# leonardsiegert/PULPo

Measured on AMD Instinct MI355X. Metric: volume-pairs/sec fwd+bwd, 160^3 fp32, higher is better.
Workload: dtype f32

## Files before the change

### include/pulpo_hip.h

```cpp
#ifndef PULPO_HIP_H
#define PULPO_HIP_H

#include <stddef.h>
#include <stdint.h>

#ifdef __cplusplus
extern "C" {
#endif

#define PULPO_ABI_VERSION 8
int pulpo_abi_version(void);
const char* pulpo_last_error(void);

size_t pulpo_conv3d_k3_packed_floats(int K, int N);
int pulpo_conv3d_k3_pack_weight(const float* w , float* wp, int Cin, int Cout, int dgrad, void* stream);
int pulpo_conv3d_k3_stat_tiles(int B, int D, int H, int W);
int pulpo_conv3d_k3_tile_config(int K, int N);
size_t pulpo_conv3d_k3_fwd_scratch_floats(int B, int D, int H, int W, int K, int N);
int pulpo_conv3d_k3_fwd(const float* in, int64_t in_bs, int64_t in_ps, int64_t in_cs, const float* wp, const float* bias, float* out,
                        int64_t out_bs, int64_t out_ps, int64_t out_cs, float* stats, float* scratch , int B,
                        int D, int H, int W, int K, int N, void* stream);
int pulpo_conv3d_k3_fwd_bn_lrelu(const float* in, int64_t in_bs, int64_t in_ps, int64_t in_cs, const float* wp, const float* bias,
                                 const float* coef, float slope, float* out, int64_t out_bs, int64_t out_ps, int64_t out_cs, float* scratch, int B,
                                 int D, int H, int W, int K, int N, void* stream);
// ... 68 lines not shown
int pulpo_heads_bwd_blocks(int B, int64_t V, int C);
int pulpo_heads_bwd(const float* h, int64_t ps, const float* Wt, const float* g0, const float* g1, const float* g2, const float* eps,
                    const float* sigma, float* dh, int64_t dps, float* partial , int nout, int B, int64_t V, int C,
                    void* stream);

int pulpo_avgpool2_fwd(const float* in, int64_t ips, float* out, int64_t ops, int B, int D, int H, int W, int C, void* stream);
int pulpo_avgpool2_bwd(const float* gout, int64_t gops, float* gin, int64_t gips, int B, int D, int H, int W, int C, void* stream);
int pulpo_avgpool2_bwd_add(const float* gout, int64_t gops, const float* add, int64_t aps, float* gin, int64_t gips, int B, int D, int H, int W,
                           int C, void* stream);
int pulpo_resize_trilinear_fwd(const float* in, const float* add, float* out, int64_t nplanes, int Di, int Hi, int Wi, int Do, int Ho, int Wo,
                               float mult, void* stream);
int pulpo_resize_trilinear_bwd(const float* gout, float* gin, int64_t nplanes, int Di, int Hi, int Wi, int Do, int Ho, int Wo, float mult,
                               void* stream);
int pulpo_resize_trilinear_scaled_fwd(const float* in, const float* add, float* out, int64_t nplanes, int Di, int Hi, int Wi, int Do, int Ho,
                                      int Wo, float scale_d, float scale_h, float scale_w, float mult, void* stream);
int pulpo_resize_trilinear_scaled_bwd(const float* gout, float* gin, int64_t nplanes, int Di, int Hi, int Wi, int Do, int Ho, int Wo,
                                      float scale_d, float scale_h, float scale_w, float mult, void* stream);
int pulpo_feedback_up2_fwd(const float* const* srcs , const int* chans , int nsrc, float* out, int64_t ops,
                           int B, int Di, int Hi, int Wi, void* stream);
int pulpo_feedback_up2_bwd(const float* gout, int64_t gops, float* const* gsrcs , const int* chans, int nsrc,
                           int B, int Di, int Hi, int Wi, void* stream);

int pulpo_warp3d_fwd(const float* df, const float* img, float* out, int B, int C, int Dg, int Hg, int Wg, int Di, int Hi, int Wi, void* stream);
int pulpo_warp_mask_fwd(const float* df, const float* mask, float* out, int B, int Dg, int Hg, int Wg, int Di, int Hi, int Wi, void* stream);
int pulpo_warp3d_bwd(const float* df, const float* img, const float* gout, float* gdf, float* gimg, int B, int C, int Dg, int Hg, int Wg, int Di,
                     int Hi, int Wi, void* stream);
int pulpo_vecint_fwd(const float* v, float* work, int B, int D, int H, int W, int nsteps, void* stream);
size_t pulpo_vecint_bwd_tmp_floats(int B, int D, int H, int W, int nsteps);
int pulpo_vecint_bwd(const float* work, const float* gout, float* gin, float* tmp , int B, int D, int H, int W,
                     int nsteps, void* stream);

int pulpo_loss_blocks(int64_t n);
int pulpo_ncc_fwd(const float* I, const float* J, float* S , float* T , float* partial, int B, int D, int H, int W,
                  int win, void* stream);
int pulpo_ncc_bwd(const float* I, const float* J, const float* S, float* T , const float* gscale, float coef, float* gJ, int B, int D,
                  int H, int W, int win, void* stream);
int pulpo_ncc_masked_fwd(const float* I, const float* J, const float* wa, const float* wb , float* S ,
                         float* T , float* partial , int B, int D, int H, int W, int win, void* stream);
int pulpo_ncc_masked_bwd(const float* I, const float* J, const float* S, const float* wa, const float* wb , float* T ,
                         const float* gscale, float coef, float* gJ, int B, int D, int H, int W, int win, void* stream);
int pulpo_masked_finish(const float* partial, int nblk, double scale, int root, double count, float* out , void* stream);
int pulpo_mind_blocks(int B, int D, int H, int W, int d);
int pulpo_mind_descriptor(const float* I, float* out , int B, int D, int H, int W, int d, float eps, void* stream);
int pulpo_mind_fwd(const float* y_true, const float* y_pred, const float* wa , const float* wb , float* partial, int B, int D,
                   int H, int W, int d, float eps, void* stream);
int pulpo_mind_bwd(const float* y_true, const float* y_pred, const float* wa , const float* wb , float* scratch ,
                   const float* gscale, float coef, float* gpred, int B, int D, int H, int W, int d, float eps, void* stream);
int pulpo_kl_fwd(const float* mu, const float* sigma, const float* mu1 , const float* sigma1 , int64_t n,
                 float* partial, void* stream);
int pulpo_kl_bwd(const float* mu, const float* sigma, const float* mu1, const float* sigma1, const float* gscale, float coef, float* gmu,
                 float* gsigma, int64_t n, void* stream);
int pulpo_l2reg_fwd(const float* df, int64_t nplanes, int D, int H, int W, float* partial, void* stream);
int pulpo_l2reg_bwd(const float* df, const float* gscale, float coef, float* gdf, int64_t nplanes, int D, int H, int W, void* stream);
int pulpo_bending_blocks(int64_t nplanes, int D, int H, int W);
int pulpo_bending_fwd(const float* df, int64_t nplanes, int D, int H, int W, float* partial, void* stream);
int pulpo_bending_bwd(const float* df, const float* gscale, float coef, float* gdf, int64_t nplanes, int D, int H, int W, void* stream);
int pulpo_weighted_sum_fwd(const float* terms, const float* weights, int n, float scale, int scaled, float* levels, float* total, void* stream);
int pulpo_weighted_sum_bwd(const float* gtotal, const float* glevels, const float* weights, int n, float scale, float* gterms, void* stream);

int pulpo_metric_blocks(int64_t n);
int pulpo_sqdiff_fwd(const float* a, const float* b, int64_t n, float* partial, void* stream);
int pulpo_sqdiff_bwd(const float* a, const float* b, const float* gscale, float coef, float* ga, int64_t n, void* stream);
int pulpo_sqdiff_masked_fwd(const float* a, const float* b, const float* wa, const float* wb ,
                            float* partial , int B, int C, int64_t V, void* stream);
int pulpo_sqdiff_masked_bwd(const float* a, const float* b, const float* wa, const float* wb , const float* gscale, float coef, float* ga,
                            int B, int C, int64_t V, void* stream);
int pulpo_dice_blocks(int64_t V);
int pulpo_dice_fwd(const float* inp, const float* tgt, int nplanes, int64_t V, float dice_factor, float* partial, double* numden, float* loss,
                   void* stream);
int pulpo_dice_bwd(const float* inp, const float* tgt, const double* numden, const float* gscale, int nplanes, int64_t V, float dice_factor,
                   float* ginp, void* stream);
int pulpo_jacdet_fwd(const float* df, float* out, double* partial , int B, int D, int H, int W, int normalize, void* stream);
int pulpo_jdetstd_finalize(const double* partial, int64_t n, float lamb, double* stat, float* loss, void* stream);
int pulpo_kl_nondiag_fwd(const float* mu, const float* sigma, int64_t nplanes, int D, int H, int W, float prior_lambda, float* partial, float* loss,
                         void* stream);
int pulpo_kl_nondiag_bwd(const float* mu, const float* sigma, const float* gscale, int64_t nplanes, int D, int H, int W, float prior_lambda,
                         float* gmu, float* gsigma, void* stream);
int pulpo_jdetstd_bwd(const float* df, const float* jdet, const double* stat, const float* gscale, float lamb, float* gdf, int B, int D, int H, int W,
                      int normalize, void* stream);

int pulpo_rmse(const float* a, const float* b, int64_t n, float* partial , float* out, void* stream);
int pulpo_dsc(const float* inp, const float* tgt, int nplanes, int64_t V, float* partial , float* out,
              void* stream);
int pulpo_percent_leq0(const float* x, int64_t n, float* partial , float* out, void* stream);
int pulpo_warp_landmarks(const float* lm , const float* df , float* out , int nlm, int nsamp,
                         int nd, int D, int H, int W, int* flag, void* stream);
int pulpo_field_quality_blocks(int B, int D, int H, int W);
size_t pulpo_field_quality_ws_bytes(int B, int D, int H, int W);
int pulpo_field_quality(const float* df, float* out , void* ws, int B, int D, int H, int W, int normalize, void* stream);

size_t pulpo_vecint_pair_scratch_floats(int B, int D, int H, int W, int nsteps);
int pulpo_vecint_pair_fwd(const float* v, float* fwd, float* inv, float* scratch , int B, int D, int H, int W, int nsteps,
                          void* stream);
size_t pulpo_inverse_consistency_ws_bytes(int B, int D, int H, int W);
int pulpo_inverse_consistency(const float* a, const float* b, float* out , void* ws, int B, int D, int H, int W, void* stream);
int pulpo_transport_points(const float* pts , const float* field , float* out , int npts,
                           int nsamp, int nd, int D, int H, int W, int* flag, void* stream);

int pulpo_affine_field(const float* theta, float* out, int B, int D, int H, int W, void* stream);
int pulpo_affine_warp_fwd(const float* theta, const float* img, float* out, int B, int C, int Dg, int Hg, int Wg, int Di, int Hi, int Wi, void* stream);
size_t pulpo_affine_warp_bwd_ws_bytes(int B, int Dg, int Hg, int Wg);
int pulpo_affine_warp_bwd(const float* theta, const float* img, const float* gout, float* gtheta , void* ws, int B, int C, int Dg, int Hg,
                          int Wg, int Di, int Hi, int Wi, void* stream);
int pulpo_affine_compose(const float* theta, const float* df, float* out, int B, int Dg, int Hg, int Wg, int Di, int Hi, int Wi, void* stream);

int pulpo_mc_moments_update(const float* sample, float* mean, float* m2, int64_t n, int k, void* stream);
int pulpo_mc_moments_std(const float* m2, const float* scale , float* out , int B, int C, int64_t V, int k, void* stream);

size_t pulpo_warp_labels_ws_bytes(int B, int C);
int pulpo_warp_labels(const float* df, const void* labels, int ldt, int C, const void* target , float* onehot ,
                      void* amax , float* dice , float* mean , float* m2 ,
                      int k, void* ws, int* flag, int B, int Dg, int Hg, int Wg, int Di, int Hi, int Wi, void* stream);
int pulpo_labels_check(const void* labels, int ldt, int64_t n, int C, int* flag, void* stream);
int pulpo_warp_labels_soft_dice(const float* df, const void* labels, const void* target, int ldt, int C, float* dice, float* mean, void* ws,
                                int* flag, int B, int Dg, int Hg, int Wg, int Di, int Hi, int Wi, int Dt, int Ht, int Wt, void* stream);
int pulpo_labels_from_onehot(const float* seg, void* labels, int ldt, int B, int C, int64_t V, void* stream);
int pulpo_map_ncc_blocks(int64_t n);
int pulpo_map_ncc(const float* a, const float* b, int64_t n, double* partial, double* out, void* stream);
int pulpo_label_dice_fwd(const float* df, const void* labels, const void* target, int ldt, int C, float dice_factor, float* loss, float* dice,
                         float* coef, void* ws, int* flag, int B, int Dg, int Hg, int Wg, int Di, int Hi, int Wi, int Dt, int Ht, int Wt,
                         void* stream);
int pulpo_label_dice_bwd(const float* df, const void* labels, const void* target, int ldt, int C, const float* coef, const float* gup, float* ddf,
                         int B, int Dg, int Hg, int Wg, int Di, int Hi, int Wi, int Dt, int Ht, int Wt, void* stream);
int pulpo_labels_pool2(const void* labels, int ldt, int C, float* out, int B, int D, int H, int W, void* stream);
int pulpo_labels_resize(const void* labels, int ldt, int C, float* out, int B, int Dt, int Ht, int Wt, int Do, int Ho, int Wo, void* stream);

#define PULPO_EDT_INF (1 << 29)
int pulpo_edt_sq(const void* mask, int* out, int B, int D, int H, int W, void* stream);
int64_t pulpo_surface_distances_bins(int D, int H, int W);
size_t pulpo_surface_distances_ws_bytes(int B, int C, int D, int H, int W);
int pulpo_surface_distances(const void* lab_a, const void* lab_b, int ldt, int C, double q, float* out, int* hist , void* ws, int* flag,
                            int B, int D, int H, int W, int nd, void* stream);

int pulpo_augment_apply(const float* theta, const float* phi, int spacing, int Gz, int Gy, int Gx, const float* img, float* img_out, int C,
                        const float* mask, float* mask_out, int Cm, const void* labels, void* labels_out, int ldt, const float* iparams, int iflags,
                        const float* bias, int Lz, int Ly, int Lx, const void* seed, float fill, int fill_label, int B, int D, int H, int W,
                        void* stream);
int pulpo_bspline_field(const float* phi, const float* theta, float* out, int spacing, int Gz, int Gy, int Gx, int B, int D, int H, int W, void* stream);
int pulpo_philox4x32(const void* counters, const void* key, void* out, int64_t n, void* stream);

int pulpo_adam_step(float* p, const float* g, float* m, float* v, int64_t n, float lr, double beta1, double beta2, float eps, int step, float gscale,
                    void* stream);
int pulpo_anchored_adam_step(float* p, const float* g, float* m, float* v, const float* mean, const float* prec, int64_t n, float lr, double beta1,
                             double beta2, float eps, int step, float* partial, void* stream);

size_t pulpo_conv3d_k3_packed_wino3_floats(int K, int N);
int pulpo_conv3d_k3_pack_weight_wino3(const float* w , float* wp, int Cin, int Cout, int dgrad, void* stream);
int pulpo_conv3d_k3_fwd_wino3(const float* in, int64_t in_bs, int64_t in_ps, int64_t in_cs, const float* wp, const float* bias, const float* coef,
                              float slope, float* out, int64_t out_bs, int64_t out_ps, int64_t out_cs, float* stats, int B, int D, int H, int W, int K,
                              int N, void* stream);
int pulpo_conv3d_k3_dgrad_wino3_bnred(const float* in, int64_t in_bs, int64_t in_ps, int64_t in_cs, const float* wp, float* out, int64_t out_bs,
                                      int64_t out_ps, const float* bn_y, int64_t bn_y_bs, int64_t bn_y_ps, const float* bn_coef, float slope, float* part,
                                      int B, int D, int H, int W, int K, int N, void* stream);

int pulpo_conv3d_k3_fwd_bf16_t(const void* in, int64_t in_bs, int64_t in_ps, int64_t in_cs, const uint16_t* wp, const float* bias, void* out,
                               int64_t out_bs, int64_t out_ps, int64_t out_cs, int dt, float* stats, float* scratch, int B, int D, int H, int W,
                               int K, int N, void* stream);
int pulpo_conv3d_k3_fwd_bn_lrelu_bf16_t(const void* in, int64_t in_bs, int64_t in_ps, int64_t in_cs, const uint16_t* wp, const float* bias,
                                        const float* coef, float slope, void* out, int64_t out_bs, int64_t out_ps, int64_t out_cs, int dt,
                                        float* scratch, int B, int D, int H, int W, int K, int N, void* stream);
int pulpo_conv3d_k3_wgrad_bf16_t(const void* in, int64_t in_bs, int64_t in_ps, int64_t in_cs, const void* dy, int64_t dy_bs, int64_t dy_ps,
                                 int64_t dy_cs, int dt, float* dw, int accumulate, float* scratch, int B, int D, int H, int W, int Cin, int Cout,
                                 void* stream);
int pulpo_bn_lrelu_apply_t(const void* y, int y_dt, int64_t yps, void* z, int z_dt, int64_t zps, const float* coef, int64_t npix, int C, float slope,
                           void* stream);
int pulpo_bn_lrelu_apply_pool2_t(const void* y, int y_dt, int64_t yps, void* z , int z_dt, int64_t zps,
                                 void* pooled , int64_t pps,
                                 const float* coef, int B, int D, int H, int W, int C, float slope, void* stream);
int pulpo_bn_lrelu_bwd_reduce_t(const void* dz, int dz_dt, int64_t dzps, const void* y, int y_dt, int64_t yps, const float* coef, int64_t npix, int C,
                                float slope, float* partial, void* stream);
int pulpo_bn_lrelu_bwd_apply_t(const void* dz, int dz_dt, int64_t dzps, const void* y, int y_dt, int64_t yps, const float* coef, const double* totd,
                               void* dy , int64_t dyps, int64_t npix, int C, float slope, float* partial2, void* stream);
int pulpo_avgpool2_bwd_bnred_t(const void* gout, int64_t gops, const void* add, int64_t aps, void* gin, int64_t gips, int g_dt ,
                               const void* y, int y_dt, int64_t yps, const float* coef, float slope, float* partial, int B, int D, int H, int W,
                               int C, void* stream);
int pulpo_heads_fwd_t(const void* h, int h_dt, int64_t ps, const float* Wt, const float* bias, const float* eps, float* o0, float* o1, float* o2,
                      int nout, int B, int64_t V, int C, void* stream);
int pulpo_heads_bwd_t(const void* h, int h_dt, int64_t ps, const float* Wt, const float* g0, const float* g1, const float* g2, const float* eps,
                      const float* sigma, void* dh , int64_t dps, float* partial, int nout, int B, int64_t V, int C, void* stream);
int pulpo_avgpool2_fwd_t(const void* in, int64_t ips, void* out, int64_t ops, int dt, int B, int D, int H, int W, int C, void* stream);
int pulpo_avgpool2_bwd_t(const void* gout, int64_t gops, const void* add , int64_t aps, void* gin, int64_t gips, int dt, int B, int D,
                         int H, int W, int C, void* stream);
int pulpo_feedback_up2_fwd_t(const float* const* srcs , const int* chans , int nsrc, void* out,
                             int dt, int64_t ops, int B, int Di, int Hi, int Wi, void* stream);
int pulpo_feedback_up2_bwd_t(const void* gout, int dt, int64_t gops, float* const* gsrcs , const int* chans,
                             int nsrc, int B, int Di, int Hi, int Wi, void* stream);

int pulpo_conv3d_k3_wgrad_bn_rows(int B, int D, int H, int W, int Cout);
int pulpo_conv3d_k3_wgrad_bn(const float* in, int64_t in_bs, int64_t in_ps, int64_t in_cs, const void* dz, int dz_dt, int64_t dz_bs, int64_t dz_ps,
                             const float* y, int64_t y_bs, int64_t y_ps, const float* coef, const double* totd, float slope, float* dw,
                             int accumulate, float* scratch, float* part2, int B, int D, int H, int W, int Cin, int Cout, void* stream);

int pulpo_bn_lrelu_bwd_apply_pooled_t(const void* gout, int64_t gops, const void* add , int64_t aps, int g_dt, const void* y, int y_dt,
                                      int64_t yps, const float* coef, const double* totd, void* dy , int64_t dyps, float slope,
                                      float* partial2, int B, int D, int H, int W, int C, void* stream);

int pulpo_bn_lrelu_apply_kb(const float* y, int64_t yps, float* z, int64_t zps, int64_t zkb, const float* coef, int64_t npix, int C, float slope, void* stream);
int pulpo_bn_lrelu_bwd_apply_kb_t(const void* dz, int dz_dt, int64_t dzps, int64_t dzkb, const float* y, int64_t yps, const float* coef, const double* totd,
                                  float* dy, int64_t dyps, int64_t dykb, int64_t npix, int C, float slope, float* partial2, void* stream);
int pulpo_conv3d_k3_wgrad_bn_kb(const float* in, int64_t in_bs, int64_t in_ps, int64_t in_cs, const float* dz, int64_t dz_bs, int64_t dz_ps, int64_t dz_kb,
                                const float* y, int64_t y_bs, int64_t y_ps, const float* coef, const double* totd, float slope, float* dw, int accumulate,
                                float* scratch, float* part2, int B, int D, int H, int W, int Cin, int Cout, void* stream);
int pulpo_bn_lrelu_bwd_apply_pooled_kb_t(const void* gout, int64_t gops, const void* add , int64_t aps, int g_dt, const float* y, int64_t yps,
                                         const float* coef, const double* totd, float* dy, int64_t dyps, int64_t dykb, float slope, float* partial2,
                                         int B, int D, int H, int W, int C, void* stream);
int pulpo_conv3d_k3_fwd_wino3_kb(const float* in, int64_t in_bs, int64_t in_ps, int64_t in_kb, const float* wp, const float* bias, const float* coef,
                                 float slope, float* out, int64_t out_bs, int64_t out_ps, int64_t out_kb, float* stats, int B, int D, int H, int W, int K,
                                 int N, void* stream);
int pulpo_conv3d_k3_dgrad_wino3_bnred_kb(const float* in, int64_t in_bs, int64_t in_ps, int64_t in_kb, const float* wp, float* out, int64_t out_bs,
                                         int64_t out_ps, int64_t out_kb, const float* bn_y, int64_t bn_y_bs, int64_t bn_y_ps, const float* bn_coef, float slope,
                                         float* part, int B, int D, int H, int W, int K, int N, void* stream);
int pulpo_conv3d_k3_wgrad_kb(const float* in, int64_t in_bs, int64_t in_ps, int64_t in_kb, const float* dy, int64_t dy_bs, int64_t dy_ps, int64_t dy_kb,
                             float* dw, int accumulate, float* scratch, float* slabs , int nslab, int B, int D, int H, int W, int Cin, int Cout,
                             void* stream);

int pulpo_conv3d_k3_wgrad_det_slabs(int Cin, int Cout);
int pulpo_conv3d_k3_wgrad_det(const float* in, int64_t in_bs, int64_t in_ps, int64_t in_cs, const float* dy, int64_t dy_bs, int64_t dy_ps,
                              int64_t dy_cs, float* dw, int accumulate, float* scratch, float* slabs, int nslab, int B, int D, int H, int W,
                              int Cin, int Cout, void* stream);
int pulpo_conv3d_k3_wgrad_bf16_det_t(const void* in, int64_t in_bs, int64_t in_ps, int64_t in_cs, const void* dy, int64_t dy_bs, int64_t dy_ps,
                                     int64_t dy_cs, int dt, float* dw, int accumulate, float* scratch, float* slabs, int nslab, int B, int D,
                                     int H, int W, int Cin, int Cout, void* stream);
int pulpo_resize_trilinear_scaled_bwd_det(const float* gout, float* gin, int64_t nplanes, int Di, int Hi, int Wi, int Do, int Ho, int Wo,
                                          float scale_d, float scale_h, float scale_w, float mult, void* stream);
size_t pulpo_warp3d_bwd_det_ws_bytes(int B, int C, int Di, int Hi, int Wi);
int pulpo_warp3d_bwd_det(const float* df, const float* img, const float* gout, float* gdf , float* gimg ,
                         void* ws , int B, int C, int Dg, int Hg, int Wg, int Di, int Hi, int Wi, void* stream);
size_t pulpo_vecint_bwd_det_ws_bytes(int B, int D, int H, int W, int nsteps);
int pulpo_vecint_bwd_det(const float* work, const float* gout, float* gin, void* ws , int B, int D, int H, int W,
                         int nsteps, void* stream);

int pulpo_conv3d_k3_wgrad_grid(int B, int D, int H, int W, int Cin, int Cout, int max_workgroups);
int pulpo_conv3d_k3_wgrad_wg(const float* in, int64_t in_bs, int64_t in_ps, int64_t in_cs, const float* dy, int64_t dy_bs, int64_t dy_ps,
                             int64_t dy_cs, float* dw, int accumulate, float* scratch, int B, int D, int H, int W, int Cin, int Cout, void* stream,
                             int max_workgroups);
int pulpo_conv3d_k3_wgrad_det_wg(const float* in, int64_t in_bs, int64_t in_ps, int64_t in_cs, const float* dy, int64_t dy_bs, int64_t dy_ps,
                                 int64_t dy_cs, float* dw, int accumulate, float* scratch, float* slabs, int nslab, int B, int D, int H, int W,
                                 int Cin, int Cout, void* stream, int max_workgroups);
int pulpo_conv3d_k3_wgrad_kb_wg(const float* in, int64_t in_bs, int64_t in_ps, int64_t in_kb, const float* dy, int64_t dy_bs, int64_t dy_ps, int64_t dy_kb,
                                float* dw, int accumulate, float* scratch, float* slabs , int nslab, int B, int D, int H, int W, int Cin, int Cout,
                                void* stream, int max_workgroups);

int pulpo_heads_fwd_bn_t(const float* y, int64_t ps, const float* coef, float slope, const float* Wt, const float* bias, const float* eps ,
                         float* o0, float* o1, float* o2, int nout, int B, int64_t V, int C, void* stream);
int pulpo_heads_bwd_bn_t(const float* y, int64_t ps, const float* coef, float slope, const float* Wt, const float* g0, const float* g1, const float* g2,
                         const float* eps, const float* sigma, float* partial , float* bnpart , int nout, int B,
                         int64_t V, int C, void* stream);
int pulpo_bn_lrelu_bwd_apply_heads_t(const float* y, int64_t yps, const float* coef, const double* totd, float slope, const float* Wt, const float* g0,
                                     const float* g1, const float* g2, const float* eps, const float* sigma, float* dy, int64_t dyps, float* partial2,
                                     int nout, int B, int64_t V, int C, void* stream);
int pulpo_bn_lrelu_bwd_apply_heads_kb_t(const float* y, int64_t yps, const float* coef, const double* totd, float slope, const float* Wt, const float* g0,
                                        const float* g1, const float* g2, const float* eps, const float* sigma, float* dy, int64_t dyps, int64_t dykb,
                                        float* partial2, int nout, int B, int64_t V, int C, void* stream);

#ifdef __cplusplus
}
#endif
#endif
```

### pulpo_amd/ops.py

```python
from __future__ import annotations

import collections
import contextlib
import ctypes
import os
from typing import Optional, Sequence, Tuple

import torch

from ._lib import PulpoHipError, lib

CL = torch.channels_last_3d
LRELU_SLOPE = 0.2


def _ptr(t: Optional[torch.Tensor]):
    return None if t is None else ctypes.c_void_p(t.data_ptr())


def _stream():
    return ctypes.c_void_p(torch.cuda.current_stream().cuda_stream)


def _require_gpu(*ts: Optional[torch.Tensor], act: bool = False):
# ... 164 lines not shown
    if n > 2 and not _sampled():
        return None
    ev = torch.cuda.Event(enable_timing=True)
    ev.record()
    return ev


def _hbm_end(start, name: str, nbytes: float):
    if start is None or HBM_TRACE is None:
        return
    end = torch.cuda.Event(enable_timing=True)
    end.record()
    HBM_TRACE.append((name, nbytes, start, end))


def _trace_end(start, name: str, flops: float, nbytes: float = 0.0):
    if start is None:
        return
    end = torch.cuda.Event(enable_timing=True)
    end.record()
    CONV_TRACE.append((name, flops, start, end, nbytes))


CONV_PRECISION = "fp32"
ACT_BF16 = False
CONV_ALGO = None


def set_conv_precision(precision: str, activations: str = "fp32") -> None:
    global CONV_PRECISION, ACT_BF16
    if precision not in ("fp32", "bf16"):
        raise ValueError(f"conv precision is {precision}. Not a known option.")
    if activations not in ("fp32", "bf16") or (activations == "bf16" and precision != "bf16"):
        raise ValueError(f"activation storage is {activations} with {precision} operands. Not a known option.")
    CONV_PRECISION = precision
    ACT_BF16 = activations == "bf16"


def act_dtype():
    return torch.bfloat16 if ACT_BF16 else torch.float32


DETERMINISTIC = os.environ.get("PULPO_DETERMINISTIC", "0") == "1"


def set_deterministic(on: bool = True) -> None:
    global DETERMINISTIC
    DETERMINISTIC = bool(on)


BN_REDUCE_IN_DGRAD = True
FUSE_INPUT_WGRAD = True
POOLED_BN_BACKWARD = True
FUSE_HEAD_BN = True


def _use_bf16(K: int) -> bool:
    return CONV_PRECISION == "bf16" and K > 4


_WEIGHT_EPOCH = 0


def invalidate_weight_packs() -> None:
    global _WEIGHT_EPOCH
    _WEIGHT_EPOCH += 1
    _PACK_REGISTRY.clear()


_PACK_REGISTRY: dict = {}
_PACK_TABLES: dict = {}
_UNREFRESHABLE_PACKS = False
_registrations = 0


def _register_pack(w: torch.Tensor, wp: torch.Tensor, Cin: int, Cout: int, dgrad: bool, kind: int) -> None:
    global _registrations
    import weakref
    _PACK_REGISTRY[id(wp)] = (weakref.ref(w), wp, Cin, Cout, dgrad, kind)
    _registrations += 1
    if _registrations % 64 == 0:
        for k in [k for k, e in _PACK_REGISTRY.items() if e[0]() is None]:
            del _PACK_REGISTRY[k]


def refresh_weight_packs() -> None:
    global _UNREFRESHABLE_PACKS
    if _UNREFRESHABLE_PACKS or not _PACK_REGISTRY:
        _UNREFRESHABLE_PACKS = False
        invalidate_weight_packs()
        return
    jobs = []
    device = None
    for key, (wref, wp, Cin, Cout, dgrad, kind) in list(_PACK_REGISTRY.items()):
        w = wref()
        cache = getattr(w, "_pulpo_packs", None) if w is not None else None
        if cache is None or cache[0] != (w._version, w.data_ptr(), _WEIGHT_EPOCH) or not any(v is wp for v in cache[1].values()):
            del _PACK_REGISTRY[key]
            continue
        jobs.append((w.data_ptr(), wp.data_ptr(), Cin, Cout, int(dgrad), kind))
        device = w.device
    if not jobs:
        invalidate_weight_packs()
        return
    tkey = tuple(jobs)
    table = _PACK_TABLES.get(tkey)
    if table is None:
        import struct
        raw = b"".join(struct.pack("<QQiiii", *job) for job in tkey)
        table = torch.frombuffer(bytearray(raw), dtype=torch.uint8).to(device)
        if len(_PACK_TABLES) > 4:
            _PACK_TABLES.clear()
        _PACK_TABLES[tkey] = table
    lib.call("pulpo_conv3d_k3_pack_weights_multi", _ptr(table), len(tkey), _stream())


def _pack_weight(w: torch.Tensor, dgrad: bool, shape=None, both: bool = False) -> torch.Tensor:
    if not w.is_leaf:
        return _pack_weight_now(w, dgrad, shape, register=False)
    cache = getattr(w, "_pulpo_packs", None)
    ver = (w._version, w.data_ptr(), _WEIGHT_EPOCH)
    if cache is None or cache[0] != ver:
        cache = (ver, {})
        try:
            w._pulpo_packs = cache
        except AttributeError:
            return _pack_weight_now(w, dgrad, shape, register=False)
    def key(d):
        return (d, CONV_PRECISION, CONV_ALGO, None if shape is None else tuple(shape))
    if both and key(not dgrad) not in cache[1]:
        cache[1][key(not dgrad)] = _pack_weight_now(w, not dgrad, shape)
    if key(dgrad) not in cache[1]:
        cache[1][key(dgrad)] = _pack_weight_now(w, dgrad, shape)
    return cache[1][key(dgrad)]


def _pack_weight_now(w: torch.Tensor, dgrad: bool, shape=None, register: bool = True) -> torch.Tensor:
    Cout, Cin = w.shape[0], w.shape[1]
    K, N = (Cout, Cin) if dgrad else (Cin, Cout)
    global _UNREFRESHABLE_PACKS
    if _use_bf16(K):
        wp = torch.empty(lib.query("pulpo_conv3d_k3_packed_bf16_elems", K, N), device=w.device, dtype=torch.int16)
        lib.call("pulpo_conv3d_k3_pack_weight_bf16", _ptr(w.contiguous()), _ptr(wp), Cin, Cout, int(dgrad), _stream())
        wp._pulpo_algo = "bf16"
        if register:
            if w.is_contiguous():
                _register_pack(w, wp, Cin, Cout, dgrad, 3)
            else:
                _UNREFRESHABLE_PACKS = True
        return wp
    algo = lib.query("pulpo_conv3d_k3_algo", *shape, K, N) if shape is not None else 0
    if CONV_ALGO is not None and algo != 0:
        algo = {"direct": 0, "wino2": 2, "wino3": algo}[CONV_ALGO]
    if algo == 3:
        wp = torch.empty(lib.query("pulpo_conv3d_k3_packed_wino3_floats", K, N), device=w.device, dtype=torch.float32)
        lib.call("pulpo_conv3d_k3_pack_weight_wino3", _ptr(w.contiguous()), _ptr(wp), Cin, Cout, int(dgrad), _stream())
        wp._pulpo_algo = "wino3"
        if register:
            if w.is_contiguous():
                _register_pack(w, wp, Cin, Cout, dgrad, 4)
            else:
                _UNREFRESHABLE_PACKS = True
        return wp
    if algo == 2:
        wp = torch.empty(lib.query("pulpo_conv3d_k3_packed_wino2_floats", K, N), device=w.device, dtype=torch.float32)
        lib.call("pulpo_conv3d_k3_pack_weight_wino2", _ptr(w.contiguous()), _ptr(wp), Cin, Cout, int(dgrad), _stream())
        wp._pulpo_algo = "wino2"
        if register:
            if w.is_contiguous():
                _register_pack(w, wp, Cin, Cout, dgrad, 2)
            else:
                _UNREFRESHABLE_PACKS = True
        return wp
    wp = torch.empty(lib.query("pulpo_conv3d_k3_packed_floats", K, N), device=w.device, dtype=torch.float32)
    lib.call("pulpo_conv3d_k3_pack_weight", _ptr(w.contiguous()), _ptr(wp), Cin, Cout, int(dgrad), _stream())
    wp._pulpo_algo = "direct"
    if register:
        if w.is_contiguous():
            _register_pack(w, wp, Cin, Cout, dgrad, 0)
        else:
            _UNREFRESHABLE_PACKS = True
    return wp


def _conv_raw(x: torch.Tensor, wp: torch.Tensor, bias: Optional[torch.Tensor], out: torch.Tensor, K: int, N: int,
              stats: Optional[torch.Tensor], coef: Optional[torch.Tensor] = None):
    B, _, D, H, W = _dims5(x)
    ob, op, oc = (0, 0, 1) if is_blocked(out) else grid_strides(out)
    algo = getattr(wp, "_pulpo_algo", "bf16" if wp.dtype == torch.int16 else "direct")
    if isinstance(x, _BlockedGrad) or is_blocked(x) or is_blocked(out):
        xt, xb_, xp_, xkb, xblk = _opnd(x)
        ot, ob_, op_, okb, oblk = _opnd(out)
        if algo != "wino3" or (not oblk and not _vec4(out)) or (not xblk and grid_strides(x)[2] != 1):
            raise PulpoHipError("conv3d on channel-blocked tensors: F(2x2x2,3x3x3) kernel, channels-last or blocked fp32 operands only")
        t0 = _trace_begin()
        lib.call("pulpo_conv3d_k3_fwd_wino3_kb", _ptr(xt), xb_, xp_, xkb, _ptr(wp), _ptr(bias), _ptr(coef), LRELU_SLOPE, _ptr(ot), ob_, op_, okb, _ptr(stats),
                 B, D, H, W, K, N, _stream())
        _trace_end(t0, "conv3d_k3_wino3_mfma<false>", 54.0 * K * N * B * D * H * W, 4.0 * (K + N) * B * D * H * W)
        return
    xb, xp, xc = grid_strides(x)
    bf16 = algo == "bf16"
    vec_ok = _vec4(x, K)
    if algo == "wino3":
        if not vec_ok:
            x = _packed_cl(x)
            xb, xp, xc = grid_strides(x)
        if not _vec4(out):
            raise PulpoHipError("conv3d (F(2x2x2,3x3x3) kernel): the result must be channels-last and 16-byte aligned")
        t0 = _trace_begin()
        lib.call("pulpo_conv3d_k3_fwd_wino3", _ptr(x), xb, xp, xc, _ptr(wp), _ptr(bias), _ptr(coef), LRELU_SLOPE, _ptr(out), ob, op, oc, _ptr(stats),
                 B, D, H, W, K, N, _stream())
        _trace_end(t0, "conv3d_k3_wino3_mfma<false>", 54.0 * K * N * B * D * H * W, 4.0 * (K + N) * B * D * H * W)
        return
    if algo == "wino2":
        if (D % 4 or D * H * W < 8000) and not vec_ok:
            x = _packed_cl(x)
            xb, xp, xc = grid_strides(x)
            vec_ok = True
        nscr = lib.query("pulpo_conv3d_k3_fwd_wino2_scratch_floats", B, D, H, W, K, N)
        scratch = torch.empty(nscr, device=x.device, dtype=torch.float32) if nscr else None
        t0 = _trace_begin()
        lib.call("pulpo_conv3d_k3_fwd_wino2", _ptr(x), xb, xp, xc, _ptr(wp), _ptr(bias), _ptr(coef), LRELU_SLOPE, _ptr(out), ob, op, oc, _ptr(stats),
                 _ptr(scratch), B, D, H, W, K, N, _stream())
        kname = f"conv3d_k3_wino2_mfma<{'true' if vec_ok else 'false'}>"
        if vec_ok and t0 is not None and lib.query("pulpo_conv3d_k3_wino2_pipelined", D, H, W, K, xp):
            kname = "conv3d_k3_wino2p_mfma<false>"
        _trace_end(t0, kname, 54.0 * K * N * B * D * H * W, 4.0 * (K + N) * B * D * H * W)
        return
    sfx = "_bf16" if bf16 else ""
    nscr = lib.query(f"pulpo_conv3d_k3_fwd{sfx}_scratch_floats", B, D, H, W, K, N)
    scratch = torch.empty(nscr, device=x.device, dtype=torch.float32) if nscr else None
    t0 = _trace_begin()
    if bf16:
        if x.dtype != out.dtype:
            raise PulpoHipError(f"conv3d (bf16 operands): input {x.dtype} and output {out.dtype} must share one storage type")
        if coef is None:
            lib.call("pulpo_conv3d_k3_fwd_bf16_t", _ptr(x), xb, xp, xc, _ptr(wp), _ptr(bias), _ptr(out), ob, op, oc, _dt(x), _ptr(stats), _ptr(scratch),
                     B, D, H, W, K, N, _stream())
        else:
            lib.call("pulpo_conv3d_k3_fwd_bn_lrelu_bf16_t", _ptr(x), xb, xp, xc, _ptr(wp), _ptr(bias), _ptr(coef), LRELU_SLOPE, _ptr(out), ob, op, oc,
                     _dt(x), _ptr(scratch), B, D, H, W, K, N, _stream())
    elif coef is None:
        lib.call("pulpo_conv3d_k3_fwd", _ptr(x), xb, xp, xc, _ptr(wp), _ptr(bias), _ptr(out), ob, op, oc, _ptr(stats), _ptr(scratch), B, D, H,
                 W, K, N, _stream())
    else:
        lib.call("pulpo_conv3d_k3_fwd_bn_lrelu", _ptr(x), xb, xp, xc, _ptr(wp), _ptr(bias), _ptr(coef), LRELU_SLOPE, _ptr(out), ob, op, oc,
                 _ptr(scratch), B, D, H, W, K, N, _stream())
    if t0 is not None:
        if bf16:
            name = f"conv3d_k3_mfma_bf16<{64 if N % 64 == 0 else 32},{'true' if vec_ok else 'false'}>"
        else:
            cfg = lib.query("pulpo_conv3d_k3_tile_config", K, N)
            name = f"conv3d_k3_mfma<{cfg // 1000},{cfg % 1000},{'true' if vec_ok and cfg // 1000 >= 16 else 'false'}>"
        _trace_end(t0, name, 54.0 * K * N * B * D * H * W, (_esize(x) * K + _esize(out) * N) * B * D * H * W)


_JOB_TABLES: dict = {}


def _persistent_buffer(owner: torch.Tensor, name: str, numel: int, zero: bool) -> torch.Tensor:
    buf = getattr(owner, name, None)
    if buf is None or buf.numel() != numel or buf.device != owner.device:
        buf = (torch.zeros if zero else torch.empty)(numel, device=owner.device, dtype=torch.float32)
        setattr(owner, name, buf)
    return buf


def _defer_grad_job(buf: torch.Tensor, dst: torch.Tensor, kind: int, a: int, b: int, c: int, byte_offset: int = 0) -> None:
    _PASS.jobs.append((buf.data_ptr() + byte_offset, dst.data_ptr(), kind, a, b, c))
    if not (_PASS.keep and _PASS.keep[-1] is buf):
        _PASS.keep.append(buf)


def _pending_src(buf: torch.Tensor) -> bool:
    p_ = buf.data_ptr()
    return any(job[0] == p_ for job in _PASS.jobs)


def flush_param_grads() -> None:
    bp = _PASS
    if not bp.jobs:
        return
    key = tuple(bp.jobs)
    table = _JOB_TABLES.get(key)
    if table is None:
        import struct
        raw = b"".join(struct.pack("<QQiiii", *job) for job in key)
        table = torch.frombuffer(bytearray(raw), dtype=torch.uint8).to(bp.keep[0].device)
        if len(_JOB_TABLES) > 8:
            _JOB_TABLES.clear()
        _JOB_TABLES[key] = table
    lib.call("pulpo_grad_finish_multi", _ptr(table), len(key), _stream())
    bp.jobs.clear()
    bp.keep.clear()


def reset_param_grad_buffers(module: Optional[torch.nn.Module] = None) -> None:
    for pending in (_PASS.jobs, _PASS.keep, _PASS.bn_parts):
        pending.clear()
    if module is not None:
        for p_ in module.parameters():
            for name in ("_pulpo_wgrad_scratch", "_pulpo_dbias_part", "_pulpo_dbias_part_in", "_pulpo_heads_part"):
                if hasattr(p_, name):
                    delattr(p_, name)


BLOCKED_DY = os.environ.get("PULPO_BLOCKED_DY", "1") != "0"
BLOCKED_DY_MIN_VOXELS = int(os.environ.get("PULPO_BLOCKED_DY_MIN_VOXELS", str(64 ** 3)))
BLOCKED_DY_HITS = 0


class _BlockedGrad:
    __slots__ = ("buf", "shape", "bs", "ps", "kb", "dtype", "device")

    def __init__(self, B, C, D, H, W, dev, buf=None):
        self.buf = torch.empty(B * C * D * H * W, device=dev, dtype=torch.float32) if buf is None else buf
        self.shape = (B, C, D, H, W)
        self.ps, self.bs, self.kb = 8, D * H * W * 8, B * D * H * W * 8
        self.dtype, self.device = torch.float32, self.buf.device

    @classmethod
    def of(cls, t6: torch.Tensor):
        B, C, D, H, W = blocked_shape(t6)
        return cls(B, C, D, H, W, t6.device, buf=t6)

    def to_cl(self) -> torch.Tensor:
        B, C, D, H, W = self.shape
        return self.buf.view(C // 8, B, D, H, W, 8).permute(1, 0, 5, 2, 3, 4).reshape(B, C, D, H, W).contiguous(memory_format=CL)


BLOCKED_Z = os.environ.get("PULPO_BLOCKED_Z", "0") == "1"
BLOCKED_Z_MIN_VOXELS = int(os.environ.get("PULPO_BLOCKED_Z_MIN_VOXELS", str(64 ** 3)))
BLOCKED_Z_HITS = 0


def is_blocked(t) -> bool:
    return isinstance(t, torch.Tensor) and t.dim() == 6


def blocked_shape(t: torch.Tensor):
    Cb, B, D, H, W, e = t.shape
    if e != 8:
        raise PulpoHipError(f"a six-dimensional activation must be channel-blocked (C / 8, B, D, H, W, 8), got {tuple(t.shape)}")
    return B, Cb * 8, D, H, W


def blocked_to_cl(t: torch.Tensor) -> torch.Tensor:
    B, C, D, H, W = blocked_shape(t)
    return t.permute(1, 0, 5, 2, 3, 4).reshape(B, C, D, H, W).contiguous(memory_format=CL)


def cl_to_blocked(t: torch.Tensor) -> torch.Tensor:
    B, C, D, H, W = t.shape
    return t.permute(0, 2, 3, 4, 1).reshape(B, D, H, W, C // 8, 8).permute(4, 0, 1, 2, 3, 5).contiguous()


def _opnd(t):
    if isinstance(t, _BlockedGrad):
        return t.buf, t.bs, t.ps, t.kb, True
    if t.dim() == 6:
        B, C, D, H, W = blocked_shape(t)
        return t, D * H * W * 8, 8, B * D * H * W * 8, True
    b, p, c = grid_strides(t)
    return t, b, p, 8, False

# ... 2362 lines not shown
```

Before: 39.91.

## Add three-stage Winograd F(2,3) GEMM forward path for small deep conv layers

Adds a new forward conv path for small spatial grids (125-1000 Winograd tiles) with wide channels. It splits the work into three kernels: an input transform kernel writes 64 transformed planes to scratch, an MFMA batched GEMM multiplies them per plane, and an output kernel applies the inverse transform, bias, optional BN+LeakyReLU and batch statistics. The goal is to replace the fused wino2 kernel on these deep, low-resolution layers where it likely underfills the GPU. The cost is large scratch traffic through global memory and two extra kernel launches. Weights are packed in the wino3 format and the path is chosen automatically when the eligibility query passes.

```diff
diff --git a/include/pulpo_hip.h b/include/pulpo_hip.h
--- a/include/pulpo_hip.h
+++ b/include/pulpo_hip.h
@@ -244,6 +244,11 @@
 int pulpo_conv3d_k3_dgrad_wino3_bnred(const float* in, int64_t in_bs, int64_t in_ps, int64_t in_cs, const float* wp, float* out, int64_t out_bs,
                                       int64_t out_ps, const float* bn_y, int64_t bn_y_bs, int64_t bn_y_ps, const float* bn_coef, float slope, float* part,
                                       int B, int D, int H, int W, int K, int N, void* stream);
+int pulpo_conv3d_k3_wino3g_ok(int B, int D, int H, int W, int K, int N);
+size_t pulpo_conv3d_k3_fwd_wino3g_scratch_floats(int B, int D, int H, int W, int K, int N);
+int pulpo_conv3d_k3_fwd_wino3g(const float* in, int64_t in_bs, int64_t in_ps, int64_t in_cs, const float* wp, const float* bias, const float* coef,
+                               float slope, float* out, int64_t out_bs, int64_t out_ps, int64_t out_cs, float* stats, float* scratch, int B, int D,
+                               int H, int W, int K, int N, void* stream);
 
 int pulpo_conv3d_k3_fwd_bf16_t(const void* in, int64_t in_bs, int64_t in_ps, int64_t in_cs, const uint16_t* wp, const float* bias, void* out,
                                int64_t out_bs, int64_t out_ps, int64_t out_cs, int dt, float* stats, float* scratch, int B, int D, int H, int W,
diff --git a/pulpo_amd/csrc/conv3d_wino3g.hip b/pulpo_amd/csrc/conv3d_wino3g.hip
--- /dev/null
+++ b/pulpo_amd/csrc/conv3d_wino3g.hip
@@ -0,0 +1,281 @@
+#include "conv_shared.h"
+#include "head_bn.h"
+
+PULPO_API int pulpo_conv3d_k3_stat_tiles(int B, int D, int H, int W);
+PULPO_API int pulpo_conv3d_k3_algo(int B, int D, int H, int W, int K, int N);
+
+namespace {
+
+using namespace pulpo_conv;
+
+constexpr int G_BM = 128;
+constexpr int G_BK = 32;
+constexpr int G_LS = G_BK + 4;
+
+__device__ __forceinline__ void wino3g_bt(float d0, float d1, float d2, float d3, float& t0, float& t1, float& t2, float& t3) {
+    t0 = d0 - d2; t1 = d1 + d2; t2 = d2 - d1; t3 = d1 - d3;
+}
+
+__global__ __launch_bounds__(256) void wino3g_input_kernel(const float* __restrict__ in, long in_bs, long in_ps, long in_cs, float* __restrict__ V, int D,
+                                                           int H, int W, int K, long nrows, long rows_pad) {
+    const long e = blockIdx.x * 256L + threadIdx.x;
+    const long plane = rows_pad * K;
+    if (e >= plane) return;
+    const long row = e / K;
+    const int k = (int)(e - row * K);
+    float d[4][4][4];
+    const int W2 = W >> 1, H2 = H >> 1, D2 = D >> 1;
+    const bool live = row < nrows;
+    long q = live ? row : 0;
+    const int bx = (int)(q % W2); q /= W2;
+    const int by = (int)(q % H2); q /= H2;
+    const int bz = (int)(q % D2);
+    const long b = q / D2;
+    const float* src = in + b * in_bs + (long)k * in_cs;
+#pragma unroll
+    for (int z = 0; z < 4; ++z) {
+        const int iz = 2 * bz - 1 + z;
+#pragma unroll
+        for (int y = 0; y < 4; ++y) {
+            const int iy = 2 * by - 1 + y;
+            const bool rowok = live && (unsigned)iz < (unsigned)D && (unsigned)iy < (unsigned)H;
+#pragma unroll
+            for (int x = 0; x < 4; ++x) {
+                const int ix = 2 * bx - 1 + x;
+                d[z][y][x] = (rowok && (unsigned)ix < (unsigned)W) ? src[((long)(iz * H + iy) * W + ix) * in_ps] : 0.f;
+            }
+        }
+    }
+#pragma unroll
+    for (int z = 0; z < 4; ++z)
+#pragma unroll
+        for (int y = 0; y < 4; ++y) wino3g_bt(d[z][y][0], d[z][y][1], d[z][y][2], d[z][y][3], d[z][y][0], d[z][y][1], d[z][y][2], d[z][y][3]);
+#pragma unroll
+    for (int z = 0; z < 4; ++z)
+#pragma unroll
+        for (int x = 0; x < 4; ++x) wino3g_bt(d[z][0][x], d[z][1][x], d[z][2][x], d[z][3][x], d[z][0][x], d[z][1][x], d[z][2][x], d[z][3][x]);
+#pragma unroll
+    for (int y = 0; y < 4; ++y)
+#pragma unroll
+        for (int x = 0; x < 4; ++x) wino3g_bt(d[0][y][x], d[1][y][x], d[2][y][x], d[3][y][x], d[0][y][x], d[1][y][x], d[2][y][x], d[3][y][x]);
+#pragma unroll
+    for (int z = 0; z < 4; ++z)
+#pragma unroll
+        for (int y = 0; y < 4; ++y)
+#pragma unroll
+            for (int x = 0; x < 4; ++x) V[(long)(z * 16 + y * 4 + x) * plane + e] = d[z][y][x];
+}
+
+}
+
+template <int RN>
+__global__ __launch_bounds__(256) __attribute__((amdgpu_waves_per_eu(4, 4))) void conv3d_k3_wino3_gemm(const float* __restrict__ V, const float* __restrict__ U, float* __restrict__ M, long rows_pad,
+                                                            int K, int N, int NPad, int nrt, int nct) {
+    constexpr int BN = RN * 32;
+    __shared__ __attribute__((aligned(16))) float As[G_BM * G_LS];
+    __shared__ __attribute__((aligned(16))) float Bs[BN * G_LS];
+    const int tid = threadIdx.x, lane = tid & 63, wave = tid >> 6;
+    const int i = lane & 31, kk = lane >> 5;
+    const int bid = pulpo::xcd_remap(blockIdx.x, gridDim.x);
+    const int ct = bid % nct;
+    const int rt = (bid / nct) % nrt;
+    const int p = bid / (nct * nrt);
+    const float* Vp = V + ((long)p * rows_pad + (long)rt * G_BM) * K;
+    const float* Up = U + ((long)p * NPad + ct * BN) * 8;
+    const long chunk_stride = 64L * NPad * 8;
+    const int nchunk = K >> 3;
+    const int nstep = (nchunk + 3) >> 2;
+
+    float4 pa[4], pb[RN];
+    auto fetch = [&](int s) {
+#pragma unroll
+        for (int j = 0; j < 4; ++j) {
+            const int idx = tid + 256 * j;
+            const int q = idx & 7, r = idx >> 3;
+            const int k = s * G_BK + 4 * q;
+            pa[j] = k < K ? *reinterpret_cast<const float4*>(Vp + (long)r * K + k) : make_float4(0.f, 0.f, 0.f, 0.f);
+        }
+#pragma unroll
+        for (int j = 0; j < RN; ++j) {
+            const int idx = tid + 256 * j;
+            const int h = idx & 1, n = (idx >> 1) % BN, cc = idx / (2 * BN);
+            const int chunk = s * 4 + cc;
+            pb[j] = (chunk < nchunk && ct * BN + n < NPad) ? *reinterpret_cast<const float4*>(Up + chunk * chunk_stride + n * 8 + 4 * h)
+                                                           : make_float4(0.f, 0.f, 0.f, 0.f);
+        }
+    };
+    auto stage = [&]() {
+#pragma unroll
+        for (int j = 0; j < 4; ++j) {
+            const int idx = tid + 256 * j;
+            *reinterpret_cast<float4*>(As + (idx >> 3) * G_LS + 4 * (idx & 7)) = pa[j];
+        }
+#pragma unroll
+        for (int j = 0; j < RN; ++j) {
+            const int idx = tid + 256 * j;
+            const int h = idx & 1, n = (idx >> 1) % BN, cc = idx / (2 * BN);
+            *reinterpret_cast<float4*>(Bs + n * G_LS + cc * 8 + 4 * h) = pb[j];
+        }
+    };
+
+    f32x16 acc[RN];
+#pragma unroll
+    for (int t = 0; t < RN; ++t)
+#pragma unroll
+        for (int r = 0; r < 16; ++r) acc[t][r] = 0.f;
+
+    fetch(0);
+    for (int s = 0; s < nstep; ++s) {
+        stage();
+        __syncthreads();
+        if (s + 1 < nstep) fetch(s + 1);
+        const float* ar = As + (wave * 32 + i) * G_LS + 4 * kk;
+        const float* br = Bs + i * G_LS + 4 * kk;
+#pragma unroll
+        for (int g = 0; g < 4; ++g) {
+            const float4 a4 = *reinterpret_cast<const float4*>(ar + g * 8);
+            float4 b4[RN];
+#pragma unroll
+            for (int t = 0; t < RN; ++t) b4[t] = *reinterpret_cast<const float4*>(br + t * 32 * G_LS + g * 8);
+#pragma unroll
+            for (int t = 0; t < RN; ++t) acc[t] = __builtin_amdgcn_mfma_f32_32x32x2f32(a4.x, b4[t].x, acc[t], 0, 0, 0);
+#pragma unroll
+            for (int t = 0; t < RN; ++t) acc[t] = __builtin_amdgcn_mfma_f32_32x32x2f32(a4.y, b4[t].y, acc[t], 0, 0, 0);
+#pragma unroll
+            for (int t = 0; t < RN; ++t) acc[t] = __builtin_amdgcn_mfma_f32_32x32x2f32(a4.z, b4[t].z, acc[t], 0, 0, 0);
+#pragma unroll
+            for (int t = 0; t < RN; ++t) acc[t] = __builtin_amdgcn_mfma_f32_32x32x2f32(a4.w, b4[t].w, acc[t], 0, 0, 0);
+        }
+        __syncthreads();
+    }
+    float* Mp = M + ((long)p * rows_pad + (long)rt * G_BM + wave * 32) * N;
+#pragma unroll
+    for (int t = 0; t < RN; ++t) {
+        const int n = ct * BN + t * 32 + i;
+        if (n < N) {
+#pragma unroll
+            for (int r = 0; r < 16; ++r) Mp[(long)((r & 3) + 8 * (r >> 2) + 4 * kk) * N + n] = acc[t][r];
+        }
+    }
+}
+
+namespace {
+
+__global__ __launch_bounds__(256) void wino3g_output_kernel(const float* __restrict__ M, const float* __restrict__ bias, const float* __restrict__ coef,
+                                                            float slope, float* __restrict__ out, long out_bs, long out_ps, long out_cs,
+                                                            float* __restrict__ stats, int D, int H, int W, int N, long nblk, long rows_pad, int nrow) {
+    __shared__ float red[2][256];
+    const int r = blockIdx.x, c = blockIdx.y * 32 + (threadIdx.x & 31), bl = threadIdx.x >> 5;
+    const long b0 = nblk * r / nrow, b1 = nblk * (r + 1) / nrow;
+    const bool cok = c < N;
+    const float bv = (cok && bias != nullptr) ? bias[c] : 0.f;
+    const bool fuse = cok && coef != nullptr;
+    const float fsc = fuse ? coef[2 * N + c] : 1.f, fsh = fuse ? coef[3 * N + c] : 0.f;
+    const int W2 = W >> 1, H2 = H >> 1, D2 = D >> 1;
+    const long plane = rows_pad * N;
+    float s = 0.f, sq = 0.f;
+    if (cok)
+        for (long blk = b0 + bl; blk < b1; blk += 8) {
+            const float* m = M + blk * N + c;
+            float tz[4][2][2];
+#pragma unroll
+            for (int pz = 0; pz < 4; ++pz) {
+                float ty[4][2];
+#pragma unroll
+                for (int py = 0; py < 4; ++py) {
+                    const float* mp = m + (long)(pz * 16 + py * 4) * plane;
+                    const float m0 = mp[0], m1 = mp[plane], m2 = mp[2 * plane], m3 = mp[3 * plane];
+                    ty[py][0] = m0 + m1 + m2;
+                    ty[py][1] = m1 - m2 - m3;
+                }
+#pragma unroll
+                for (int ox = 0; ox < 2; ++ox) {
+                    tz[pz][0][ox] = ty[0][ox] + ty[1][ox] + ty[2][ox];
+                    tz[pz][1][ox] = ty[1][ox] - ty[2][ox] - ty[3][ox];
+                }
+            }
+            long q = blk;
+            const int bx = (int)(q % W2); q /= W2;
+            const int by = (int)(q % H2); q /= H2;
+            const int bz = (int)(q % D2);
+            const long b = q / D2;
+            float* o = out + b * out_bs + (long)c * out_cs;
+#pragma unroll
+            for (int oy = 0; oy < 2; ++oy)
+#pragma unroll
+                for (int ox = 0; ox < 2; ++ox) {
+                    float v[2];
+                    v[0] = tz[0][oy][ox] + tz[1][oy][ox] + tz[2][oy][ox] + bv;
+                    v[1] = tz[1][oy][ox] - tz[2][oy][ox] - tz[3][oy][ox] + bv;
+#pragma unroll
+                    for (int oz = 0; oz < 2; ++oz) {
+                        s += v[oz];
+                        sq += v[oz] * v[oz];
+                        const float w = fuse ? pulpo::bn_lrelu(v[oz], fsc, fsh, slope) : v[oz];
+                        o[((long)((2 * bz + oz) * H + 2 * by + oy) * W + 2 * bx + ox) * out_ps] = w;
+                    }
+                }
+        }
+    if (stats != nullptr) {
+        red[0][threadIdx.x] = s;
+        red[1][threadIdx.x] = sq;
+        __syncthreads();
+        if (threadIdx.x < 64) {
+            const int which = threadIdx.x >> 5, cc = threadIdx.x & 31;
+            float t = 0.f;
+#pragma unroll
+            for (int k = 0; k < 8; ++k) t += red[which][k * 32 + cc];
+            if (blockIdx.y * 32 + cc < N) stats[((long)r * 2 + which) * N + blockIdx.y * 32 + cc] = t;
+        }
+    }
+}
+
+long wino3g_blocks(int B, int D, int H, int W) { return (long)B * (D / 2) * (H / 2) * (W / 2); }
+long wino3g_rows_pad(int B, int D, int H, int W) { return (wino3g_blocks(B, D, H, W) + G_BM - 1) / G_BM * G_BM; }
+
+bool wino3g_entry_ok(int B, int D, int H, int W, int K, int N) {
+    return B > 0 && D > 0 && H > 0 && W > 0 && D % 2 == 0 && H % 2 == 0 && W % 2 == 0 && K > 0 && K % 8 == 0 && N > 0 && N % 4 == 0;
+}
+
+}
+
+PULPO_API int pulpo_conv3d_k3_wino3g_ok(int B, int D, int H, int W, int K, int N) {
+    if (!wino3g_entry_ok(B, D, H, W, K, N) || N % 32 != 0 || pulpo_conv3d_k3_algo(B, D, H, W, K, N) != 2) return 0;
+    const long blocks = wino3g_blocks(B, D, H, W);
+    return blocks >= 125 && blocks <= 1000 && std::min(K, N) >= 128;
+}
+
+PULPO_API size_t pulpo_conv3d_k3_fwd_wino3g_scratch_floats(int B, int D, int H, int W, int K, int N) {
+    if (!wino3g_entry_ok(B, D, H, W, K, N)) return 0;
+    return (size_t)64 * wino3g_rows_pad(B, D, H, W) * ((size_t)K + N);
+}
+
+PULPO_API int pulpo_conv3d_k3_fwd_wino3g(const float* in, int64_t in_bs, int64_t in_ps, int64_t in_cs, const float* wp, const float* bias,
+                                         const float* coef, float slope, float* out, int64_t out_bs, int64_t out_ps, int64_t out_cs, float* stats,
+                                         float* scratch, int B, int D, int H, int W, int K, int N, void* stream) {
+    PULPO_REQUIRE(in && wp && out && scratch, "conv3d_k3_fwd_wino3g: null pointer");
+    PULPO_REQUIRE(wino3g_entry_ok(B, D, H, W, K, N),
+                  "conv3d_k3_fwd_wino3g: shape %dx%dx%d, %d -> %d channels: even extents, K %% 8 == 0 and N %% 4 == 0 required", D, H, W, K, N);
+    PULPO_REQUIRE(!(coef && stats), "conv3d_k3_fwd_wino3g: batch statistics are not available from the fused eval-mode epilogue");
+    PULPO_REQUIRE((((uintptr_t)wp | (uintptr_t)scratch) & 15) == 0, "conv3d_k3_fwd_wino3g: packed weights and scratch must be 16-byte aligned");
+    const long nblk = wino3g_blocks(B, D, H, W), rows_pad = wino3g_rows_pad(B, D, H, W);
+    const int rn = N % 96 == 0 ? 3 : 2;
+    const int nrt = (int)(rows_pad / G_BM), nct = pulpo::cdiv(N, rn * 32);
+    PULPO_REQUIRE(64L * nrt * nct < (1L << 31) && rows_pad * K < (1L << 31) * 256, "conv3d_k3_fwd_wino3g: grid too large");
+    PULPO_REQUIRE(nct * rn * 32 <= npad(N), "conv3d_k3_fwd_wino3g: column tiles exceed the weight pack");
+    hipStream_t st = (hipStream_t)stream;
+    float* V = scratch;
+    float* M = scratch + 64 * rows_pad * K;
+    hipLaunchKernelGGL(wino3g_input_kernel, dim3(pulpo::cdiv(rows_pad * K, 256)), dim3(256), 0, st, in, (long)in_bs, (long)in_ps, (long)in_cs, V, D, H, W, K,
+                       nblk, rows_pad);
+    int rc = pulpo::check_launch("wino3g_input");
+    if (rc != 0) return rc;
+    if (rn == 3) hipLaunchKernelGGL((conv3d_k3_wino3_gemm<3>), dim3(64 * nrt * nct), dim3(256), 0, st, V, wp, M, rows_pad, K, N, npad(N), nrt, nct);
+    else hipLaunchKernelGGL((conv3d_k3_wino3_gemm<2>), dim3(64 * nrt * nct), dim3(256), 0, st, V, wp, M, rows_pad, K, N, npad(N), nrt, nct);
+    rc = pulpo::check_launch("conv3d_k3_wino3_gemm");
+    if (rc != 0) return rc;
+    const int nrow = pulpo_conv3d_k3_stat_tiles(B, D, H, W);
+    hipLaunchKernelGGL(wino3g_output_kernel, dim3(nrow, pulpo::cdiv(N, 32)), dim3(256), 0, st, M, bias, coef, slope, out, (long)out_bs, (long)out_ps,
+                       (long)out_cs, stats, D, H, W, N, nblk, rows_pad, nrow);
+    return pulpo::check_launch("wino3g_output");
+}
diff --git a/pulpo_amd/ops.py b/pulpo_amd/ops.py
--- a/pulpo_amd/ops.py
+++ b/pulpo_amd/ops.py
@@ -340,10 +340,11 @@
     algo = lib.query("pulpo_conv3d_k3_algo", *shape, K, N) if shape is not None else 0
     if CONV_ALGO is not None and algo != 0:
         algo = {"direct": 0, "wino2": 2, "wino3": algo}[CONV_ALGO]
-    if algo == 3:
+    gemm = algo == 2 and CONV_ALGO in (None, "wino3") and bool(lib.query("pulpo_conv3d_k3_wino3g_ok", *shape, K, N))
+    if algo == 3 or gemm:
         wp = torch.empty(lib.query("pulpo_conv3d_k3_packed_wino3_floats", K, N), device=w.device, dtype=torch.float32)
         lib.call("pulpo_conv3d_k3_pack_weight_wino3", _ptr(w.contiguous()), _ptr(wp), Cin, Cout, int(dgrad), _stream())
-        wp._pulpo_algo = "wino3"
+        wp._pulpo_algo = "wino3g" if gemm else "wino3"
         if register:
             if w.is_contiguous():
                 _register_pack(w, wp, Cin, Cout, dgrad, 4)
@@ -399,6 +400,13 @@
         lib.call("pulpo_conv3d_k3_fwd_wino3", _ptr(x), xb, xp, xc, _ptr(wp), _ptr(bias), _ptr(coef), LRELU_SLOPE, _ptr(out), ob, op, oc, _ptr(stats),
                  B, D, H, W, K, N, _stream())
         _trace_end(t0, "conv3d_k3_wino3_mfma<false>", 54.0 * K * N * B * D * H * W, 4.0 * (K + N) * B * D * H * W)
+        return
+    if algo == "wino3g":
+        scratch = torch.empty(lib.query("pulpo_conv3d_k3_fwd_wino3g_scratch_floats", B, D, H, W, K, N), device=x.device, dtype=torch.float32)
+        t0 = _trace_begin()
+        lib.call("pulpo_conv3d_k3_fwd_wino3g", _ptr(x), xb, xp, xc, _ptr(wp), _ptr(bias), _ptr(coef), LRELU_SLOPE, _ptr(out), ob, op, oc, _ptr(stats),
+                 _ptr(scratch), B, D, H, W, K, N, _stream())
+        _trace_end(t0, f"conv3d_k3_wino3_gemm<{3 if N % 96 == 0 else 2}>", 54.0 * K * N * B * D * H * W, 4.0 * (K + N) * B * D * H * W)
         return
     if algo == "wino2":
         if (D % 4 or D * H * W < 8000) and not vec_ok:
```

After: 40.80 (median of 6 runs). +2.2%, better.
